# IXarea/LittleGAN

Hardware: AMD Instinct MI355X
Metric: 128x128 CelebA-shaped images/sec (G+D+Adj step) (higher is better)
Workload: dtype bf16; 1 GPU; C3: 128x128x3 synthetic CelebA, batch 256/GPU, bf16 MFMA conv/transposed-conv + Adjuster branch; global_batch=256, per_gpu_batch=256, image=128, cond_dim=40, parallelism=dp1, launch=eager launches

## Files before the change

### littlegan_amd/csrc/conv_down3.hip

```cpp
#include <type_traits>
#include "lg_internal.h"

namespace {

constexpr int TH = 8, TW = 16;
constexpr int HH = 2 * TH + 3;
constexpr int ROWB = 48;
constexpr int KC = 16;
constexpr int NTAP = 25;
template <bool PAIR>
struct D3L {
  static constexpr int HWH = PAIR ? 10 : 18, HWP = PAIR ? 43 : 2 * HWH;
  static constexpr int NROWS = HH * HWP;
  static constexpr int HB = NROWS * ROWB;
  static constexpr int NPIECE = NROWS * 2;
  static constexpr int PPT = (NPIECE + 255) / 256;
  static constexpr int SRED_OFF = 2 * HB;
  static constexpr int SBIAS_OFF = 2 * HB + 256;
  static constexpr int LDS_BYTES = 2 * HB + 256 + 512;
};
#ifndef LG_D3_DBG
#define LG_D3_DBG 0
#endif
constexpr int DBG = LG_D3_DBG;
constexpr int RING = 10;
constexpr int ADEPTH = 2;
constexpr int STAGGER = 6;
constexpr int BLOCKS_PER_CU = 2;

struct D3Params {
  const __bf16* src;
  const char* wp;
  const float* bias;
  __bf16* out;
  double* spart;
  int B, Hs, Ws, Cs, Hm, Wm, N, N32, KB;
  int tpi_x, tpi, ntn, nitems, nparts;
  LgNormFuse nf;
  const float* nstats;
  float nalpha;
  const __bf16* gsrc;
  const float* bcoef;
  unsigned long long* clk;
};

__device__ __forceinline__ int pix32(int r) {
  const int q = r >> 2, lo = r & 3;
  const int odd = (q ^ (q >> 1) ^ (q >> 2)) & 1;
  const int rank = odd ? ((q == 1) ? 0 : (q == 2) ? 1 : (q == 4) ? 2 : 3) : ((q == 0) ? 0 : (q == 3) ? 1 : (q == 5) ? 2 : 3);
  return odd * 16 + rank * 4 + lo;
}

template <bool PAIR>
constexpr int toff_bytes(int t) {
  return ((t / 5) * D3L<PAIR>::HWP + ((t % 5) >> 1) + ((t % 5) & 1) * D3L<PAIR>::HWH) * ROWB;
}

template <bool STATS, bool FUSE = false, bool PAIR = false, int NW = 128, int NORM = 0>
__global__ __launch_bounds__(256, 2) void conv_down3_kernel(const D3Params p) {
  static_assert(!(STATS && FUSE), "forward moments and backward sums are never needed together");
  static_assert(NORM != 1 || (STATS && NW == 128 && !PAIR), "the normalising form exists for the forward passes with fused moments, 8 x 16 tiles");
  static_assert(NORM != 2 || (!STATS && !PAIR && NW == 64), "the backward-normalising form exists for the 64-column data gradients on 8 x 16 tiles");
  static_assert(NW == 128 || (NW == 64 && !PAIR), "tile widths");
  constexpr int NWV = NW / 32, NI = NW / 32;
  constexpr int PPR = NW / 8, NQ = 128 * PPR / 256;
  using L = D3L<PAIR>;
  constexpr int HWH = L::HWH, HWP = L::HWP, HB = L::HB, NPIECE = L::NPIECE, PPT = L::PPT, SRED_OFF = L::SRED_OFF, SBIAS_OFF = L::SBIAS_OFF;
  extern __shared__ __attribute__((aligned(16))) char smem[];
  double* sred = reinterpret_cast<double*>(smem + SRED_OFF);
  const int tid = threadIdx.x, lane = tid & 63, r = lane & 31, h = lane >> 5;
  const int wid = __builtin_amdgcn_readfirstlane(tid >> 6);
  const int wn = wid % NWV, wm = wid / NWV;
  const int G = gridDim.x;
  const int nchunk = p.Cs / KC;
  const int nx = G < 8 ? G : 8, xcd = (int)blockIdx.x % nx, xidx = (int)blockIdx.x / nx;
  const int lb = lg_xcd_remap(blockIdx.x, G);
  const int nfull = p.nitems / G, nrem = p.nitems - nfull * G;
  const int rcnt = (nrem - xcd + nx - 1) / nx;
  const int rstart = nfull * G + xcd * (nrem / nx) + (xcd < nrem % nx ? xcd : nrem % nx);
  const int nmine = nfull + (xidx < rcnt ? 1 : 0);
  const int total = nmine * nchunk;
  const unsigned long long clk_t0 = __builtin_amdgcn_s_memtime(), clk_r0 = __builtin_amdgcn_s_memrealtime();
  int pl[PPT], pyx[PPT];
#pragma unroll
  for (int u = 0; u < PPT; ++u) {
    const int q = tid + u * 256;
    if constexpr (PAIR) {
      pl[u] = -1; pyx[u] = 0;
      if (q < NPIECE) {
        const int row = q >> 1, hy = row / HWP, hxp = row - hy * HWP;
        pl[u] = row * ROWB + (q & 1) * 16;
        const int sm = hxp >= 24, j2 = hxp - 24 * sm, odd = j2 >= HWH, hx = 2 * (j2 - odd * HWH) + odd;
        pyx[u] = (hxp < 20 || hxp >= 24) && hx < 2 * 8 + 3 ? (hy << 8) | (sm << 7) | hx : (0x7fff << 8);
      }
    } else {
      constexpr int PPROW = 2 * (2 * TW + 3);
      pl[u] = -1; pyx[u] = (0x7fff << 8);
      if (q < HH * PPROW) {
        const int hy = q / PPROW, rem = q - hy * PPROW, hx = rem >> 1;
        const int hxp = (hx & 1) ? HWH + (hx >> 1) : (hx >> 1);
        pl[u] = (hy * HWP + hxp) * ROWB + (rem & 1) * 16;
        pyx[u] = (hy << 8) | hx;
      }
    }
  }
  const int half8 = (tid & 1) * 8;

  int abase[NI];
#pragma unroll
  for (int i = 0; i < NI; ++i) {
    const int m = (wm * NI + i) * 32 + pix32(r);
    const int col = m & 15;
    abase[i] = (2 * (m >> 4) * HWP + (PAIR ? col + 16 * (col >> 3) : col)) * ROWB + h * 16;
  }

  struct Item { int n, y0, x0, tn; };
  auto decode = [&](int k) {
    const int item = k == nfull ? rstart + xidx : lb + k * G;
    Item it;
    it.tn = item % p.ntn;
    const int tm = item / p.ntn;
    if constexpr (PAIR) { it.n = 2 * tm; it.y0 = 0; it.x0 = 0; return it; }
    it.n = tm / p.tpi;
    const int tt = tm - it.n * p.tpi;
    it.y0 = (tt / p.tpi_x) * TH; it.x0 = (tt % p.tpi_x) * TW;
    return it;
  };
  constexpr unsigned OOB = 0x80000000u;
  const int sample_elems = p.Hs * p.Ws * p.Cs;
  unsigned hoff[PPT];
  float nmu0 = 0.f, nml0 = 0.f, nna0 = 0.f, nnb0 = 0.f;
  LgBwdCoef bco{};
  auto set_item = [&](const Item& it) __attribute__((always_inline)) {
    if constexpr (NORM == 1) {
      const lg_const_f32p sp = lg_as_const(p.nstats + (long long)it.n * 8);
      nmu0 = lg_uniform(sp[0]); nna0 = lg_uniform(sp[2]); nnb0 = lg_uniform(sp[3]); nml0 = lg_uniform(sp[4]);
    }
    if constexpr (NORM == 2) {
      const lg_const_f32p sp = lg_as_const(p.bcoef + (long long)it.n * 8);
      bco.mu = lg_uniform(sp[0]); bco.mul = lg_uniform(sp[1]); bco.a = lg_uniform(sp[2]); bco.b = lg_uniform(sp[3]);
      bco.m1 = lg_uniform(sp[4]); bco.m2 = lg_uniform(sp[5]); bco.m1l = lg_uniform(sp[6]); bco.m2l = lg_uniform(sp[7]);
    }
#pragma unroll
    for (int u = 0; u < PPT; ++u) {
      const int sy = 2 * it.y0 - 1 + (pyx[u] >> 8), sx = 2 * it.x0 - 1 + (pyx[u] & (PAIR ? 127 : 255));
      const int sl = PAIR ? (pyx[u] >> 7) & 1 : 0;
      const bool ok = pl[u] >= 0 && (unsigned)sy < (unsigned)p.Hs && (unsigned)sx < (unsigned)p.Ws;
      hoff[u] = ok ? (unsigned)((((sl * p.Hs + sy) * p.Ws + sx) * p.Cs + half8) * 2) : OOB;
    }
  };
  auto issue = [&](const Item& it, int c0, u32x4 (&v)[PPT]) __attribute__((always_inline)) {
    const __amdgpu_buffer_rsrc_t rs = __builtin_amdgcn_make_buffer_rsrc(
        const_cast<__bf16*>(p.src + (long long)it.n * sample_elems), 0, (PAIR ? 2 : 1) * sample_elems * 2, 0x00027000);
#pragma unroll
    for (int u = 0; u < PPT; ++u) v[u] = __builtin_bit_cast(u32x4, __builtin_amdgcn_raw_buffer_load_b128(rs, hoff[u] + (unsigned)c0 * 2u, 0, 0));
  };
  auto issue_g = [&](const Item& it, int c0, u32x4 (&v)[NORM == 2 ? PPT : 1]) __attribute__((always_inline)) {
    if constexpr (NORM == 2) {
      const __amdgpu_buffer_rsrc_t rs = __builtin_amdgcn_make_buffer_rsrc(
          const_cast<__bf16*>(p.gsrc + (long long)it.n * sample_elems), 0, sample_elems * 2, 0x00027000);
#pragma unroll
      for (int u = 0; u < PPT; ++u) v[u] = __builtin_bit_cast(u32x4, __builtin_amdgcn_raw_buffer_load_b128(rs, hoff[u] + (unsigned)c0 * 2u, 0, 0));
    }
  };
  u32x4 gv[NORM == 2 ? PPT : 1];
  auto commit = [&](char* buf, const u32x4 (&v)[PPT]) __attribute__((always_inline)) {
#pragma unroll
    for (int u = 0; u < PPT; ++u)
      if (pl[u] >= 0) {
        u32x4 w = v[u];
        if constexpr (NORM == 2) {
          const u32x4 dn = lg_bwdnorm8(w, gv[u], bco, p.nalpha);
          const bool inside = hoff[u] != OOB;
#pragma unroll
          for (int k = 0; k < 4; ++k) w[k] = inside ? dn[k] : 0u;
        }
        if constexpr (NORM == 1) {
          const u32x4 hn = lg_norm8(w, nmu0, nml0, nna0, nnb0, p.nalpha);
          const bool inside = hoff[u] != OOB;
#pragma unroll
          for (int k = 0; k < 4; ++k) w[k] = inside ? hn[k] : 0u;
        }
        if constexpr ((DBG & 16) != 0) {
          const float mu = p.nf.alpha, mul = 0.001f, na = 1.01f, nb = 0.02f, al = 0.3f;
#pragma unroll
          for (int k = 0; k < 4; ++k) {
            float t0 = __builtin_bit_cast(float, w[k] << 16), t1 = __builtin_bit_cast(float, w[k] & 0xffff0000u);
            t0 = na * ((t0 - mu) - mul) + nb; t1 = na * ((t1 - mu) - mul) + nb;
            t0 = fmaxf(t0, al * t0); t1 = fmaxf(t1, al * t1);
            const __bf16 h0 = (__bf16)t0, h1 = (__bf16)t1;
            const unsigned o = (unsigned)__builtin_bit_cast(unsigned short, h0) | ((unsigned)__builtin_bit_cast(unsigned short, h1) << 16);
            w[k] = pyx[u] != (0x7fff << 8) ? o : 0u;
          }
        }
        *reinterpret_cast<u32x4*>(buf + pl[u]) = w;
      }
  };
  const unsigned lane16 = lane * 16;
  const unsigned wstride = (unsigned)p.N32 * (unsigned)p.KB * 1024u;
  auto wbase = [&](int tn, int kb) {
    return p.wp + ((long long)(tn * NWV + wn) * p.KB + kb) * 1024;
  };
  auto wfrag = [&](const char* base, int t) {
    return *reinterpret_cast<const u32x4*>((base + (unsigned long long)t * wstride) + lane16);
  };

  f32x16 acc[NI];
#pragma unroll
  for (int i = 0; i < NI; ++i)
#pragma unroll
    for (int e = 0; e < 16; ++e) acc[i][e] = 0.f;
  static_assert(NTAP % RING != 0, "the slice body is instantiated for the two ring offsets 0 and NTAP % RING");
  constexpr int AD = ADEPTH;
  u32x4 bf[RING];
  u32x4 hv[PPT];

  Item cur = decode(0);
  set_item(cur);
  issue(cur, 0, hv);
  issue_g(cur, 0, gv);
#pragma unroll
  for (int t = 0; t < RING; ++t) bf[t] = wfrag(wbase(cur.tn, 0), t);
  commit(smem, hv);
  __syncthreads();

  float* sbias = reinterpret_cast<float*>(smem + SBIAS_OFF);
  auto load_bias = [&](int tn) {
    if (tid < NW) sbias[tid] = p.bias ? p.bias[tn * NW + tid] : 0.f;
  };
  load_bias(cur.tn);
  {
    if ((int)blockIdx.x >= (G + 1) / 2)
      for (int i = 0; i < STAGGER; ++i) __builtin_amdgcn_s_sleep(16);
  }
  int k = 0, c = 0;
  auto slice = [&](auto off_c, int s) {
    constexpr int OFF = decltype(off_c)::value;
    const bool more = s + 1 < total;
    const bool last_c = c + 1 == nchunk;
    Item nxt = cur;
    int c2 = c + 1;
    if (last_c) { c2 = 0; if (more) { nxt = decode(k + 1); set_item(nxt); } }
    if (!more) c2 = c;
    if constexpr (!(DBG & 4)) { issue(nxt, c2 * KC, hv); issue_g(nxt, c2 * KC, gv); }
    const char* hbuf = smem + (s & 1) * HB;
    const char* wcur = wbase(cur.tn, c);
    const char* wnxt = wbase(nxt.tn, c2);
    bf16x8 a[AD][NI];
#pragma unroll
    for (int d = 0; d + 1 < AD; ++d)
#pragma unroll
      for (int i = 0; i < NI; ++i) a[d][i] = *reinterpret_cast<const bf16x8*>(hbuf + abase[i] + toff_bytes<PAIR>(d));
    __builtin_amdgcn_sched_barrier(0);
#pragma unroll
    for (int t = 0; t < NTAP; ++t) {
      if (t + AD - 1 < NTAP) {
#pragma unroll
        for (int i = 0; i < NI; ++i)
          a[(t + AD - 1) % AD][i] = *reinterpret_cast<const bf16x8*>(hbuf + abase[i] + toff_bytes<PAIR>(t + AD - 1 < NTAP ? t + AD - 1 : 0));
      }
      const int slot = (t + OFF) % RING;
#pragma unroll
      for (int i = 0; i < NI; ++i)
        if constexpr (!(DBG & 1)) acc[i] = __builtin_amdgcn_mfma_f32_32x32x16_bf16(__builtin_bit_cast(bf16x8, bf[slot]), a[t % AD][i], acc[i], 0, 0, 0);
      if constexpr (!(DBG & 2)) {
        if (t + RING < NTAP) bf[slot] = wfrag(wcur, t + RING);
        else bf[slot] = wfrag(wnxt, t + RING - NTAP);
      }
#pragma unroll
      for (int i = 0; i < NI; ++i) {
        __builtin_amdgcn_sched_group_barrier(0x008, 1, 0);
        __builtin_amdgcn_sched_group_barrier(0x100, 1, 0);
      }
      __builtin_amdgcn_sched_group_barrier(0x020, 1, 0);
    }
    if constexpr (NORM != 0) __builtin_amdgcn_sched_barrier(0);
    commit(smem + ((s + 1) & 1) * HB, hv);
    __syncthreads();

    if (last_c && !(DBG & 8)) {
      char* C = smem + (s & 1) * HB;
      const float shift = STATS ? sbias[0] : 0.f;
      const f32x2 shift2 = {shift, shift};
      f32x2 s1v = {0.f, 0.f}, s2v = {0.f, 0.f};
      f32x4 bq[4];
#pragma unroll
      for (int g = 0; g < 4; ++g) bq[g] = *reinterpret_cast<const f32x4*>(sbias + wn * 32 + 8 * g + 4 * h);
#pragma unroll
      for (int i = 0; i < NI; ++i) {
        const int row = (wm * NI + i) * 32 + pix32(r);
#pragma unroll
        for (int g = 0; g < 4; ++g) {
          bf16x4 w;
#pragma unroll
          for (int jj = 0; jj < 2; ++jj) {
            const f32x2 v = f32x2{acc[i][4 * g + 2 * jj], acc[i][4 * g + 2 * jj + 1]} + f32x2{bq[g][2 * jj], bq[g][2 * jj + 1]};
            if constexpr (STATS) {
              const f32x2 d = v - shift2;
              s1v += d;
              s2v = __builtin_elementwise_fma(d, d, s2v);
            }
            w[2 * jj] = (__bf16)v[0]; w[2 * jj + 1] = (__bf16)v[1];
          }
          *reinterpret_cast<bf16x4*>(C + row * (NW * 2) + (((wn * 4 + g) ^ (row & (PPR - 1))) << 4) + 8 * h) = w;
        }
      }
      if constexpr (STATS) {
        const double l1 = (double)s1v[0] + (double)s1v[1], l2 = (double)s2v[0] + (double)s2v[1];
        if constexpr (PAIR) {
          const bool sb = (pix32(r) & 8) != 0;
          const double a1 = lg_wave_sum_d(sb ? 0.0 : l1), a2 = lg_wave_sum_d(sb ? 0.0 : l2);
          const double b1 = lg_wave_sum_d(sb ? l1 : 0.0), b2 = lg_wave_sum_d(sb ? l2 : 0.0);
          if (lane == 0) {
            double* q = sred + (k & 1) * 16;
            q[wid] = a1; q[4 + wid] = a2; q[8 + wid] = b1; q[12 + wid] = b2;
          }
        } else {
          const double w1 = lg_wave_sum_d(l1), w2 = lg_wave_sum_d(l2);
          if (lane == 0) { sred[(k & 1) * 16 + wid] = w1; sred[(k & 1) * 16 + 4 + wid] = w2; }
        }
      }
      const long long obase = ((long long)(cur.n * p.Hm + cur.y0) * p.Wm + cur.x0) * p.N + cur.tn * NW;
      auto pix_off = [&](int row) -> long long {
        if constexpr (PAIR) return obase + (long long)(((row >> 3) & 1) * 64 + (row >> 4) * 8 + (row & 7)) * p.N;
        else return obase + ((long long)(row >> 4) * p.Wm + (row & 15)) * p.N;
      };
      u32x4 zq[FUSE ? NQ : 1];
      (void)zq;
      if constexpr (FUSE) {
#pragma unroll
        for (int q8 = 0; q8 < NQ; ++q8) {
          const int piece = tid + q8 * 256, row = piece / PPR, j = piece % PPR;
          zq[q8] = *reinterpret_cast<const u32x4*>(p.nf.z + pix_off(row) + j * 8);
        }
      }
      __syncthreads();
      float nf1 = 0.f, nf2 = 0.f;
      (void)nf1; (void)nf2;
#pragma unroll
      for (int q8 = 0; q8 < NQ; ++q8) {
        const int piece = tid + q8 * 256, row = piece / PPR, j = piece % PPR;
        const u32x4 v = *reinterpret_cast<const u32x4*>(C + row * (NW * 2) + ((j ^ (row & (PPR - 1))) << 4));
        const long long goff = pix_off(row) + j * 8;
        *reinterpret_cast<u32x4*>(p.out + goff) = v;
        if constexpr (FUSE) {
          const lg_const_f32p sp = lg_as_const(p.nf.stats + (long long)(cur.n + (PAIR ? wid >> 1 : 0)) * 8);
          lg_nf_accum(v, zq[q8], lg_uniform(sp[0]), lg_uniform(sp[4]), lg_uniform(sp[2]), lg_uniform(sp[3]), p.nf.alpha, nf1, nf2);
        }
      }
      if constexpr (FUSE) {
        const double w1 = lg_wave_sum_d((double)nf1), w2 = lg_wave_sum_d((double)nf2);
        if (lane == 0) { sred[(k & 1) * 16 + wid] = w1; sred[(k & 1) * 16 + 4 + wid] = w2; }
      }
      if constexpr (STATS) {
        if (tid == 0) {
          const double* q = sred + (k & 1) * 16;
          if constexpr (PAIR) {
            constexpr double cnt = 64.0 * 128.0;
#pragma unroll
            for (int sm = 0; sm < 2; ++sm) {
              const double S1 = (q[8 * sm] + q[8 * sm + 1]) + (q[8 * sm + 2] + q[8 * sm + 3]);
              const double S2 = (q[8 * sm + 4] + q[8 * sm + 5]) + (q[8 * sm + 6] + q[8 * sm + 7]);
              const double md = S1 / cnt;
              double* o = p.spart + ((long long)(cur.n + sm) * p.nparts + cur.tn) * 3;
              o[0] = cnt; o[1] = (double)shift + md; o[2] = S2 - cnt * md * md;
            }
          } else {
            constexpr double cnt = 128.0 * NW;
            const double S1 = (q[0] + q[1]) + (q[2] + q[3]), S2 = (q[4] + q[5]) + (q[6] + q[7]);
            const double md = S1 / cnt;
            const int tin = (cur.y0 / TH) * p.tpi_x + cur.x0 / TW;
            double* o = p.spart + ((long long)cur.n * p.nparts + tin * p.ntn + cur.tn) * 3;
            o[0] = cnt; o[1] = (double)shift + md; o[2] = S2 - cnt * md * md;
          }
        }
      }
      __syncthreads();
      if constexpr (FUSE) {
        if (tid == 0) {
          const double* q = sred + (k & 1) * 16;
          if constexpr (PAIR) {
#pragma unroll
            for (int sm = 0; sm < 2; ++sm) {
              double* o = p.nf.part + ((long long)(cur.n + sm) * p.nparts + cur.tn) * 2;
              o[0] = q[2 * sm] + q[2 * sm + 1]; o[1] = q[4 + 2 * sm] + q[4 + 2 * sm + 1];
            }
          } else {
            const int tin = (cur.y0 / TH) * p.tpi_x + cur.x0 / TW;
            double* o = p.nf.part + ((long long)cur.n * p.nparts + tin * p.ntn + cur.tn) * 2;
            o[0] = (q[0] + q[1]) + (q[2] + q[3]); o[1] = (q[4] + q[5]) + (q[6] + q[7]);
          }
        }
      }
#pragma unroll
      for (int i = 0; i < NI; ++i)
#pragma unroll
        for (int e = 0; e < 16; ++e) acc[i][e] = 0.f;
      if (more && nxt.tn != cur.tn) load_bias(nxt.tn);
      ++k;
    }
    cur = nxt;
    c = c2;
  };
  for (int s = 0; s < total; s += 2) {
    slice(std::integral_constant<int, 0>{}, s);
    if (s + 1 < total) slice(std::integral_constant<int, NTAP % RING>{}, s + 1);
  }
  if (p.clk && wid == 0 && lane == 0) {
    const unsigned long long t1 = __builtin_amdgcn_s_memtime(), r1 = __builtin_amdgcn_s_memrealtime();
    if (t1 > clk_t0 && r1 > clk_r0) {
      atomicAdd(p.clk, t1 - clk_t0); atomicAdd(p.clk + 1, r1 - clk_r0); atomicAdd(p.clk + 2, 1ull);
    }
  }
}

}

enum D3Tiling { D3_NONE = 0, D3_PLAIN, D3_PAIR, D3_N64 };
static D3Tiling down3_tiling(int B, int Hm, int Wm, int Cs, int N) {
  static int off = -1;
  if (off < 0) off = lg_env_flag("LG_NO_DOWN3") ? 1 : 0;
  if (off || B <= 0 || Cs % KC) return D3_NONE;
  if ((long long)4 * Hm * Wm * Cs * 2 * 2 >= (1ll << 31)) return D3_NONE;
  const bool pair = Hm == 8 && Wm == 8 && B % 2 == 0;
  if (!pair && (Hm % TH || Wm % TW)) return D3_NONE;
  if (N % 128 == 0) return pair ? D3_PAIR : D3_PLAIN;
  return (N % 64 == 0 && !pair) ? D3_N64 : D3_NONE;
}
extern "C" int lg_conv_down3_supported(int B, int Hm, int Wm, int Cs, int N) { return down3_tiling(B, Hm, Wm, Cs, N) != D3_NONE ? 1 : 0; }
extern "C" int lg_conv_down3_zn_supported(int B, int Hm, int Wm, int Cs, int N) {
  return (!lg_env_flag("LG_NO_D3_NORM") && down3_tiling(B, Hm, Wm, Cs, N) == D3_PLAIN) ? 1 : 0;
}
extern "C" int lg_conv_down3_bn_supported(int B, int Hm, int Wm, int Cs, int N) {
  return (!lg_env_flag("LG_NO_D3_BWDNORM") && N == 64 && down3_tiling(B, Hm, Wm, Cs, N) == D3_N64) ? 1 : 0;
}

static int down3_launch(const void* src16, const void* wpack, const float* bias, void* out16, int B, int Hm, int Wm, int Cs, int N,
                        void* spart, size_t spart_bytes, int* nparts_out, const LgNormFuse* nf, size_t nf_bytes,
                        const float* nstats, float nalpha, void* stream, const void* g16 = nullptr, const float* bcoef = nullptr) {
  if (nparts_out) *nparts_out = 0;
  const D3Tiling tiling = down3_tiling(B, Hm, Wm, Cs, N);
  if (tiling == D3_NONE || !src16 || !wpack || !out16) return LG_ERR_UNSUPPORTED;
  const bool pair = tiling == D3_PAIR, n64 = tiling == D3_N64;
  D3Params p{};
  p.src = (const __bf16*)src16; p.wp = (const char*)wpack; p.bias = bias; p.out = (__bf16*)out16;
  p.B = B; p.Hm = Hm; p.Wm = Wm; p.Hs = 2 * Hm; p.Ws = 2 * Wm; p.Cs = Cs; p.N = N; p.N32 = N / 32; p.KB = Cs / 16;
  p.tpi_x = pair ? 1 : Wm / TW; p.tpi = pair ? 1 : p.tpi_x * (Hm / TH); p.ntn = n64 ? N / 64 : N / 128;
  const long long nitems = (long long)(pair ? B / 2 : B) * p.tpi * p.ntn;
  if (nitems <= 0 || nitems >= (1ll << 30)) return LG_ERR_UNSUPPORTED;
  p.nitems = (int)nitems; p.nparts = p.tpi * p.ntn;
  const bool fuse = nf && nf->z && nf->stats && nf->part && nparts_out && (size_t)B * p.nparts * 2 * sizeof(double) <= nf_bytes;
  const bool stats = !fuse && spart && nparts_out && (size_t)B * p.nparts * 3 * sizeof(double) <= spart_bytes;
  if (!nf && spart && nparts_out && !stats) return LG_ERR_UNSUPPORTED;
  p.spart = stats ? (double*)spart : nullptr;
  if (fuse) p.nf = *nf;
  if (nstats && (!stats || n64 || pair)) return LG_ERR_UNSUPPORTED;
  if (g16 && (!fuse || pair || nstats || !n64 || p.ntn != 1)) return LG_ERR_UNSUPPORTED;
  p.nstats = nstats; p.nalpha = nalpha;
  p.gsrc = (const __bf16*)g16; p.bcoef = bcoef;
  p.clk = lg_clock_census();
  static bool attr_set = false;
  if (!attr_set) {
    attr_set = true;
    (void)hipFuncSetAttribute(reinterpret_cast<const void*>(conv_down3_kernel<true>), hipFuncAttributeMaxDynamicSharedMemorySize, D3L<false>::LDS_BYTES);
    (void)hipFuncSetAttribute(reinterpret_cast<const void*>(conv_down3_kernel<false>), hipFuncAttributeMaxDynamicSharedMemorySize, D3L<false>::LDS_BYTES);
    (void)hipFuncSetAttribute(reinterpret_cast<const void*>((conv_down3_kernel<false, true>)), hipFuncAttributeMaxDynamicSharedMemorySize, D3L<false>::LDS_BYTES);
    (void)hipFuncSetAttribute(reinterpret_cast<const void*>((conv_down3_kernel<true, false, true>)), hipFuncAttributeMaxDynamicSharedMemorySize, D3L<true>::LDS_BYTES);
    (void)hipFuncSetAttribute(reinterpret_cast<const void*>((conv_down3_kernel<false, false, true>)), hipFuncAttributeMaxDynamicSharedMemorySize, D3L<true>::LDS_BYTES);
    (void)hipFuncSetAttribute(reinterpret_cast<const void*>((conv_down3_kernel<false, true, true>)), hipFuncAttributeMaxDynamicSharedMemorySize, D3L<true>::LDS_BYTES);
    (void)hipFuncSetAttribute(reinterpret_cast<const void*>((conv_down3_kernel<true, false, false, 64>)), hipFuncAttributeMaxDynamicSharedMemorySize, D3L<false>::LDS_BYTES);
    (void)hipFuncSetAttribute(reinterpret_cast<const void*>((conv_down3_kernel<false, false, false, 64>)), hipFuncAttributeMaxDynamicSharedMemorySize, D3L<false>::LDS_BYTES);
    (void)hipFuncSetAttribute(reinterpret_cast<const void*>((conv_down3_kernel<false, true, false, 64>)), hipFuncAttributeMaxDynamicSharedMemorySize, D3L<false>::LDS_BYTES);
    (void)hipFuncSetAttribute(reinterpret_cast<const void*>((conv_down3_kernel<true, false, false, 128, 1>)), hipFuncAttributeMaxDynamicSharedMemorySize, D3L<false>::LDS_BYTES);
    (void)hipFuncSetAttribute(reinterpret_cast<const void*>((conv_down3_kernel<false, true, false, 64, 2>)), hipFuncAttributeMaxDynamicSharedMemorySize, D3L<false>::LDS_BYTES);
  }
  const int nblk = BLOCKS_PER_CU * lg_grid_cus();
  const int grid = p.nitems < nblk ? p.nitems : nblk;
  hipStream_t st = (hipStream_t)stream;
  constexpr int LDS0 = D3L<false>::LDS_BYTES, LDS1 = D3L<true>::LDS_BYTES;
  if (nstats) {
    hipLaunchKernelGGL((conv_down3_kernel<true, false, false, 128, 1>), dim3(grid), dim3(256), LDS0, st, p);
  } else if (g16) {
    hipLaunchKernelGGL((conv_down3_kernel<false, true, false, 64, 2>), dim3(grid), dim3(256), LDS0, st, p);
  } else if (pair) {
    if (fuse) hipLaunchKernelGGL((conv_down3_kernel<false, true, true>), dim3(grid), dim3(256), LDS1, st, p);
    else if (stats) hipLaunchKernelGGL((conv_down3_kernel<true, false, true>), dim3(grid), dim3(256), LDS1, st, p);
    else hipLaunchKernelGGL((conv_down3_kernel<false, false, true>), dim3(grid), dim3(256), LDS1, st, p);
  } else if (n64) {
    if (fuse) hipLaunchKernelGGL((conv_down3_kernel<false, true, false, 64>), dim3(grid), dim3(256), LDS0, st, p);
    else if (stats) hipLaunchKernelGGL((conv_down3_kernel<true, false, false, 64>), dim3(grid), dim3(256), LDS0, st, p);
    else hipLaunchKernelGGL((conv_down3_kernel<false, false, false, 64>), dim3(grid), dim3(256), LDS0, st, p);
  } else if (fuse) hipLaunchKernelGGL((conv_down3_kernel<false, true>), dim3(grid), dim3(256), LDS0, st, p);
  else if (stats) hipLaunchKernelGGL(conv_down3_kernel<true>, dim3(grid), dim3(256), LDS0, st, p);
  else hipLaunchKernelGGL(conv_down3_kernel<false>, dim3(grid), dim3(256), LDS0, st, p);
  LG_CHECK_LAUNCH("lg_conv_down3");
  lg_note_kernel(g16 ? "conv_down3_kernel<NW=64,BWDNORM>" : nstats ? "conv_down3_kernel<NW=128,NORM>" : pair ? "conv_down3_kernel<PAIR>" : n64 ? "conv_down3_kernel<NW=64>" : "conv_down3_kernel<NW=128>");
  if (stats || fuse) *nparts_out = p.nparts;
  return LG_OK;
}

extern "C" int lg_conv_down3_nf_try(const void* src16, const void* wpack, const float* bias, void* out16, int B, int Hm, int Wm,
                                    int Cs, int N, void* spart, size_t spart_bytes, int* nparts_out, const LgNormFuse* nf,
                                    size_t nf_bytes, void* stream) {
  return down3_launch(src16, wpack, bias, out16, B, Hm, Wm, Cs, N, spart, spart_bytes, nparts_out, nf, nf_bytes, nullptr, 0.f, stream);
}
extern "C" int lg_conv_down3_try(const void* src16, const void* wpack, const float* bias, void* out16, int B, int Hm, int Wm,
                                 int Cs, int N, void* spart, size_t spart_bytes, int* nparts_out, void* stream) {
  return lg_conv_down3_nf_try(src16, wpack, bias, out16, B, Hm, Wm, Cs, N, spart, spart_bytes, nparts_out, nullptr, 0, stream);
}
extern "C" int lg_conv_down3_zn_try(const void* z16, const float* zstats, float alpha, const void* wpack, const float* bias, void* out16,
                                    int B, int Hm, int Wm, int Cs, int N, void* spart, size_t spart_bytes, int* nparts_out, void* stream) {
  if (nparts_out) *nparts_out = 0;
  if (!zstats || !spart || !nparts_out || !lg_conv_down3_zn_supported(B, Hm, Wm, Cs, N)) return LG_ERR_UNSUPPORTED;
  return down3_launch(z16, wpack, bias, out16, B, Hm, Wm, Cs, N, spart, spart_bytes, nparts_out, nullptr, 0, zstats, alpha, stream);
}
extern "C" int lg_conv_down3_bn_try(const void* z16, const void* g16, const float* bcoef, float alpha, const void* wpack, void* out16,
                                    int B, int Hm, int Wm, int Cs, int N, int* nparts_out, const LgNormFuse* nf, size_t nf_bytes,
                                    void* stream) {
  if (nparts_out) *nparts_out = 0;
  if (!g16 || !bcoef || !nf || !nparts_out || !lg_conv_down3_bn_supported(B, Hm, Wm, Cs, N)) return LG_ERR_UNSUPPORTED;
  return down3_launch(z16, wpack, nullptr, out16, B, Hm, Wm, Cs, N, nullptr, 0, nparts_out, nf, nf_bytes, nullptr, alpha, stream, g16, bcoef);
}
```

Baseline: 24440 images/sec.

## Split 64-column down-conv taps across wave pairs with LDS reduction of partial sums

For the NW=64 variant, each wave now covers all four 32-row M fragments and handles only half of the 25 taps: one wave row takes the first 13 taps, the other takes the remaining 12. Each wave keeps a smaller weight-fragment ring. At the epilogue the partial accumulators are exchanged and summed through the idle halo buffer in LDS. The goal is less redundant weight-fragment traffic per wave and fewer weight registers. In exchange there is an extra LDS exchange, a barrier, and a new output staging layout, and the tap work is unbalanced between the two halves.

Result: no change. 24410 images/sec (-0.1%).

```diff
diff --git a/littlegan_amd/csrc/conv_down3.hip b/littlegan_amd/csrc/conv_down3.hip
--- a/littlegan_amd/csrc/conv_down3.hip
+++ b/littlegan_amd/csrc/conv_down3.hip
@@ -24,6 +24,7 @@
 #endif
 constexpr int DBG = LG_D3_DBG;
 constexpr int RING = 10;
+constexpr int RING64 = 7;
 constexpr int ADEPTH = 2;
 constexpr int STAGGER = 6;
 constexpr int BLOCKS_PER_CU = 2;
@@ -62,9 +63,12 @@
   static_assert(NORM != 1 || (STATS && NW == 128 && !PAIR), "the normalising form exists for the forward passes with fused moments, 8 x 16 tiles");
   static_assert(NORM != 2 || (!STATS && !PAIR && NW == 64), "the backward-normalising form exists for the 64-column data gradients on 8 x 16 tiles");
   static_assert(NW == 128 || (NW == 64 && !PAIR), "tile widths");
-  constexpr int NWV = NW / 32, NI = NW / 32;
+  constexpr bool SPLIT = NW == 64;
+  constexpr int NWV = NW / 32, NI = 4;
   constexpr int PPR = NW / 8, NQ = 128 * PPR / 256;
+  constexpr int QUARTER = 64 * 32 * 4;
   using L = D3L<PAIR>;
+  static_assert(!SPLIT || 4 * QUARTER <= L::HB, "the merge buffer is the idle halo buffer");
   constexpr int HWH = L::HWH, HWP = L::HWP, HB = L::HB, NPIECE = L::NPIECE, PPT = L::PPT, SRED_OFF = L::SRED_OFF, SBIAS_OFF = L::SBIAS_OFF;
   extern __shared__ __attribute__((aligned(16))) char smem[];
   double* sred = reinterpret_cast<double*>(smem + SRED_OFF);
@@ -109,9 +113,13 @@
   int abase[NI];
 #pragma unroll
   for (int i = 0; i < NI; ++i) {
-    const int m = (wm * NI + i) * 32 + pix32(r);
+    const int m = ((SPLIT ? 0 : wm) * NI + i) * 32 + pix32(r);
     const int col = m & 15;
     abase[i] = (2 * (m >> 4) * HWP + (PAIR ? col + 16 * (col >> 3) : col)) * ROWB + h * 16;
+  }
+  if constexpr (SPLIT) {
+#pragma unroll
+    for (int i = 1; i < NI; ++i) abase[i] = abase[0] + i * (4 * HWP * ROWB);
   }
 
   struct Item { int n, y0, x0, tn; };
@@ -141,8 +149,14 @@
       bco.mu = lg_uniform(sp[0]); bco.mul = lg_uniform(sp[1]); bco.a = lg_uniform(sp[2]); bco.b = lg_uniform(sp[3]);
       bco.m1 = lg_uniform(sp[4]); bco.m2 = lg_uniform(sp[5]); bco.m1l = lg_uniform(sp[6]); bco.m2l = lg_uniform(sp[7]);
     }
+    int tq = tid;
+    if constexpr (SPLIT) asm volatile("" : "+v"(tq));
 #pragma unroll
     for (int u = 0; u < PPT; ++u) {
+      if constexpr (SPLIT) {
+        const int q = tq + u * 256, hy = q / (2 * (2 * TW + 3));
+        pyx[u] = (hy << 8) | ((q - hy * (2 * (2 * TW + 3))) >> 1);
+      }
       const int sy = 2 * it.y0 - 1 + (pyx[u] >> 8), sx = 2 * it.x0 - 1 + (pyx[u] & (PAIR ? 127 : 255));
       const int sl = PAIR ? (pyx[u] >> 7) & 1 : 0;
       const bool ok = pl[u] >= 0 && (unsigned)sy < (unsigned)p.Hs && (unsigned)sx < (unsigned)p.Ws;
@@ -212,15 +226,27 @@
     for (int e = 0; e < 16; ++e) acc[i][e] = 0.f;
   static_assert(NTAP % RING != 0, "the slice body is instantiated for the two ring offsets 0 and NTAP % RING");
   constexpr int AD = ADEPTH;
-  u32x4 bf[RING];
+  constexpr int NT0 = (NTAP + 1) / 2, NT1 = NTAP - NT0;
+  constexpr int SR0 = RING64, SR1 = SR0 - 1;
+  u32x4 bf[SPLIT ? SR0 : RING];
   u32x4 hv[PPT];
 
   Item cur = decode(0);
   set_item(cur);
   issue(cur, 0, hv);
   issue_g(cur, 0, gv);
-#pragma unroll
-  for (int t = 0; t < RING; ++t) bf[t] = wfrag(wbase(cur.tn, 0), t);
+  if constexpr (SPLIT) {
+    if (wm == 0) {
+#pragma unroll
+      for (int j = 0; j < SR0; ++j) bf[j] = wfrag(wbase(cur.tn, 0), j);
+    } else {
+#pragma unroll
+      for (int j = 0; j < SR1; ++j) bf[j] = wfrag(wbase(cur.tn, 0), NT0 + j);
+    }
+  } else {
+#pragma unroll
+    for (int t = 0; t < RING; ++t) bf[t] = wfrag(wbase(cur.tn, 0), t);
+  }
   commit(smem, hv);
   __syncthreads();
 
@@ -246,33 +272,65 @@
     const char* hbuf = smem + (s & 1) * HB;
     const char* wcur = wbase(cur.tn, c);
     const char* wnxt = wbase(nxt.tn, c2);
-    bf16x8 a[AD][NI];
-#pragma unroll
-    for (int d = 0; d + 1 < AD; ++d)
-#pragma unroll
-      for (int i = 0; i < NI; ++i) a[d][i] = *reinterpret_cast<const bf16x8*>(hbuf + abase[i] + toff_bytes<PAIR>(d));
-    __builtin_amdgcn_sched_barrier(0);
-#pragma unroll
-    for (int t = 0; t < NTAP; ++t) {
-      if (t + AD - 1 < NTAP) {
+    if constexpr (SPLIT) {
+      constexpr int T0 = OFF ? NT0 : 0, NT = OFF ? NT1 : NT0, SR = OFF ? SR1 : SR0;
+      bf16x8 a[AD][NI];
+#pragma unroll
+      for (int d = 0; d + 1 < AD; ++d)
+#pragma unroll
+        for (int i = 0; i < NI; ++i) a[d][i] = *reinterpret_cast<const bf16x8*>(hbuf + abase[i] + toff_bytes<PAIR>(T0 + d));
+      __builtin_amdgcn_sched_barrier(0);
+#pragma unroll
+      for (int j = 0; j < NT; ++j) {
+        if (j + AD - 1 < NT) {
+#pragma unroll
+          for (int i = 0; i < NI; ++i)
+            a[(j + AD - 1) % AD][i] = *reinterpret_cast<const bf16x8*>(hbuf + abase[i] + toff_bytes<PAIR>(j + AD - 1 < NT ? T0 + j + AD - 1 : 0));
+        }
+        const int slot = j % SR;
 #pragma unroll
         for (int i = 0; i < NI; ++i)
-          a[(t + AD - 1) % AD][i] = *reinterpret_cast<const bf16x8*>(hbuf + abase[i] + toff_bytes<PAIR>(t + AD - 1 < NTAP ? t + AD - 1 : 0));
-      }
-      const int slot = (t + OFF) % RING;
-#pragma unroll
-      for (int i = 0; i < NI; ++i)
-        if constexpr (!(DBG & 1)) acc[i] = __builtin_amdgcn_mfma_f32_32x32x16_bf16(__builtin_bit_cast(bf16x8, bf[slot]), a[t % AD][i], acc[i], 0, 0, 0);
-      if constexpr (!(DBG & 2)) {
-        if (t + RING < NTAP) bf[slot] = wfrag(wcur, t + RING);
-        else bf[slot] = wfrag(wnxt, t + RING - NTAP);
-      }
-#pragma unroll
-      for (int i = 0; i < NI; ++i) {
-        __builtin_amdgcn_sched_group_barrier(0x008, 1, 0);
-        __builtin_amdgcn_sched_group_barrier(0x100, 1, 0);
-      }
-      __builtin_amdgcn_sched_group_barrier(0x020, 1, 0);
+          if constexpr (!(DBG & 1)) acc[i] = __builtin_amdgcn_mfma_f32_32x32x16_bf16(__builtin_bit_cast(bf16x8, bf[slot]), a[j % AD][i], acc[i], 0, 0, 0);
+        if constexpr (!(DBG & 2)) {
+          if (j + SR < NT) bf[slot] = wfrag(wcur, T0 + j + SR);
+          else bf[slot] = wfrag(wnxt, T0 + slot);
+        }
+#pragma unroll
+        for (int i = 0; i < NI; ++i) {
+          __builtin_amdgcn_sched_group_barrier(0x008, 1, 0);
+          __builtin_amdgcn_sched_group_barrier(0x100, 1, 0);
+        }
+        __builtin_amdgcn_sched_group_barrier(0x020, 1, 0);
+      }
+    } else {
+      bf16x8 a[AD][NI];
+#pragma unroll
+      for (int d = 0; d + 1 < AD; ++d)
+#pragma unroll
+        for (int i = 0; i < NI; ++i) a[d][i] = *reinterpret_cast<const bf16x8*>(hbuf + abase[i] + toff_bytes<PAIR>(d));
+      __builtin_amdgcn_sched_barrier(0);
+#pragma unroll
+      for (int t = 0; t < NTAP; ++t) {
+        if (t + AD - 1 < NTAP) {
+#pragma unroll
+          for (int i = 0; i < NI; ++i)
+            a[(t + AD - 1) % AD][i] = *reinterpret_cast<const bf16x8*>(hbuf + abase[i] + toff_bytes<PAIR>(t + AD - 1 < NTAP ? t + AD - 1 : 0));
+        }
+        const int slot = (t + OFF) % RING;
+#pragma unroll
+        for (int i = 0; i < NI; ++i)
+          if constexpr (!(DBG & 1)) acc[i] = __builtin_amdgcn_mfma_f32_32x32x16_bf16(__builtin_bit_cast(bf16x8, bf[slot]), a[t % AD][i], acc[i], 0, 0, 0);
+        if constexpr (!(DBG & 2)) {
+          if (t + RING < NTAP) bf[slot] = wfrag(wcur, t + RING);
+          else bf[slot] = wfrag(wnxt, t + RING - NTAP);
+        }
+#pragma unroll
+        for (int i = 0; i < NI; ++i) {
+          __builtin_amdgcn_sched_group_barrier(0x008, 1, 0);
+          __builtin_amdgcn_sched_group_barrier(0x100, 1, 0);
+        }
+        __builtin_amdgcn_sched_group_barrier(0x020, 1, 0);
+      }
     }
     if constexpr (NORM != 0) __builtin_amdgcn_sched_barrier(0);
     commit(smem + ((s + 1) & 1) * HB, hv);
@@ -280,6 +338,28 @@
 
     if (last_c && !(DBG & 8)) {
       char* C = smem + (s & 1) * HB;
+      constexpr int I0 = SPLIT ? 2 * OFF : 0, NIE = SPLIT ? 2 : NI;
+      if constexpr (SPLIT) {
+        char* give = C + (wn * 2 + OFF) * QUARTER + lane16;
+        const char* take = C + (wn * 2 + (1 - OFF)) * QUARTER + lane16;
+#pragma unroll
+        for (int ii = 0; ii < 2; ++ii)
+#pragma unroll
+          for (int g = 0; g < 4; ++g) {
+            const int i = 2 * (1 - OFF) + ii;
+            *reinterpret_cast<f32x4*>(give + (ii * 4 + g) * 1024) = f32x4{acc[i][4 * g], acc[i][4 * g + 1], acc[i][4 * g + 2], acc[i][4 * g + 3]};
+          }
+        __syncthreads();
+#pragma unroll
+        for (int ii = 0; ii < 2; ++ii)
+#pragma unroll
+          for (int g = 0; g < 4; ++g) {
+            const f32x4 v = *reinterpret_cast<const f32x4*>(take + (ii * 4 + g) * 1024);
+#pragma unroll
+            for (int e = 0; e < 4; ++e)
+              acc[I0 + ii][4 * g + e] = OFF == 0 ? acc[I0 + ii][4 * g + e] + v[e] : v[e] + acc[I0 + ii][4 * g + e];
+          }
+      }
       const float shift = STATS ? sbias[0] : 0.f;
       const f32x2 shift2 = {shift, shift};
       f32x2 s1v = {0.f, 0.f}, s2v = {0.f, 0.f};
@@ -287,8 +367,8 @@
 #pragma unroll
       for (int g = 0; g < 4; ++g) bq[g] = *reinterpret_cast<const f32x4*>(sbias + wn * 32 + 8 * g + 4 * h);
 #pragma unroll
-      for (int i = 0; i < NI; ++i) {
-        const int row = (wm * NI + i) * 32 + pix32(r);
+      for (int i = I0; i < I0 + NIE; ++i) {
+        const int row = ((SPLIT ? 0 : wm) * NI + i) * 32 + pix32(r);
 #pragma unroll
         for (int g = 0; g < 4; ++g) {
           bf16x4 w;
@@ -302,7 +382,11 @@
             }
             w[2 * jj] = (__bf16)v[0]; w[2 * jj + 1] = (__bf16)v[1];
           }
-          *reinterpret_cast<bf16x4*>(C + row * (NW * 2) + (((wn * 4 + g) ^ (row & (PPR - 1))) << 4) + 8 * h) = w;
+          if constexpr (SPLIT) {
+            *reinterpret_cast<bf16x4*>(C + (wn * 2 + (1 - OFF)) * QUARTER + wn * 128 + (row & 63) * 64 + ((g ^ ((row >> 2) & 3)) << 4) + 8 * h) = w;
+          } else {
+            *reinterpret_cast<bf16x4*>(C + row * (NW * 2) + (((wn * 4 + g) ^ (row & (PPR - 1))) << 4) + 8 * h) = w;
+          }
         }
       }
       if constexpr (STATS) {
@@ -340,7 +424,8 @@
 #pragma unroll
       for (int q8 = 0; q8 < NQ; ++q8) {
         const int piece = tid + q8 * 256, row = piece / PPR, j = piece % PPR;
-        const u32x4 v = *reinterpret_cast<const u32x4*>(C + row * (NW * 2) + ((j ^ (row & (PPR - 1))) << 4));
+        const u32x4 v = SPLIT ? *reinterpret_cast<const u32x4*>(C + ((j >> 2) * 2 + (1 - (row >> 6))) * QUARTER + (j >> 2) * 128 + (row & 63) * 64 + (((j & 3) ^ ((row >> 2) & 3)) << 4))
+                              : *reinterpret_cast<const u32x4*>(C + row * (NW * 2) + ((j ^ (row & (PPR - 1))) << 4));
         const long long goff = pix_off(row) + j * 8;
         *reinterpret_cast<u32x4*>(p.out + goff) = v;
         if constexpr (FUSE) {
@@ -402,9 +487,14 @@
     cur = nxt;
     c = c2;
   };
-  for (int s = 0; s < total; s += 2) {
-    slice(std::integral_constant<int, 0>{}, s);
-    if (s + 1 < total) slice(std::integral_constant<int, NTAP % RING>{}, s + 1);
+  if constexpr (SPLIT) {
+    if (wm == 0) for (int s = 0; s < total; ++s) slice(std::integral_constant<int, 0>{}, s);
+    else for (int s = 0; s < total; ++s) slice(std::integral_constant<int, 1>{}, s);
+  } else {
+    for (int s = 0; s < total; s += 2) {
+      slice(std::integral_constant<int, 0>{}, s);
+      if (s + 1 < total) slice(std::integral_constant<int, NTAP % RING>{}, s + 1);
+    }
   }
   if (p.clk && wid == 0 && lane == 0) {
     const unsigned long long t1 = __builtin_amdgcn_s_memtime(), r1 = __builtin_amdgcn_s_memrealtime();
```
